# griffin-h/lightcurve_fitting

Measured on AMD Instinct MI355X. Metric: walker-steps/sec (emcee ensemble), higher is better.
Workload: dtype f64

## Files before the change

### lightcurve_fitting_amd/csrc/lcf_device.h

```cpp
#pragma once
#ifndef __HIPCC_RTC__
#include <hip/hip_runtime.h>
#include <stdint.h>
#else
typedef __hip_internal::int32_t int32_t;
typedef __hip_internal::uint32_t uint32_t;
typedef __hip_internal::int64_t int64_t;
typedef __hip_internal::uint64_t uint64_t;
#ifndef INFINITY
#define INFINITY __builtin_huge_valf()
#endif
#endif

namespace lcf {

constexpr int kBlock = 256;
constexpr int kMaxParts = 8;
constexpr int kFewEpochs = 128;
constexpr int kTargetGroups = 4096;
constexpr int kNCoef = 8;
constexpr int kMaxDim = 16;
constexpr int kLdsFiltMax = 64;
constexpr int kLdsTabMax = 3700;
constexpr int kMaxPeers = 8;
// ... 394 lines not shown
                const double Tk = c[1] * exp((2. * eps1 - 0.5) * lt);
                const double E = (c[3] == c[3]) ? exp(fma(alpha, lt, c[3])) : 0.;
                const double L = c[2] * exp(-2. * eps2 * lt - E);
                if (!(L >= 0.)) {
                    pref = qnan();
                } else if (Tk > 0. && Tk < kTmax) {
                    const double i1 = inv_temperature(Tk), i2 = i1 * i1;
                    T = Tk;
                    invT = i1;
                    pref = kC3sq * L * i2 * i2;
                }
            } else if (t < 0. && c[4] != 0.) {
                pref = qnan();
            }
            break;
        }
        case kShockCooling4: {
            const double tt = t / c[3];
            double P1 = 0., P2 = 0., P3 = 0., P4 = 0.;
            if (tt > 0.) {
                const double ltt = log(tt);
                P1 = exp(-4. / 3. * ltt);
                P2 = exp(-0.17 * ltt);
                P3 = exp(-1. / 3. * ltt);
                P4 = exp(-0.45 * ltt);
            }
            const double u = k[1] * t / c[4];
            const double E = u > 0. ? pow(u, k[2]) : 0.;
            const double L = c[2] * (P1 + k[0] * exp(-E) * P2);
            const double Tk = c[1] * fmin(0.97 * P3, P4);
            if (!(L >= 0.)) {
                pref = qnan();
            } else if (Tk > 0. && Tk < kTmax) {
                const double i1 = inv_temperature(Tk), i2 = i1 * i1;
                T = Tk;
                invT = i1;
                pref = kC3sq * L * i2 * i2;
            }
            break;
        }
        case kCompanion:
        case kCompanion2:
        case kCompanion3: {
            if (t > 0.) {
                const double lt = log(t);
                if (lt > -9.5916 && lt < 10.06) {
                    const double Tk = c[1] * exp(-74. / 144. * lt);
                    if (Tk > 0. && Tk < kTmax) {
                        T = Tk;
                        invT = inv_temperature(Tk);
                        pref = c[2] * exp(14. / 9. * lt);
                    }
                }
            }
            break;
        }
        case kBlackbody:
            if (c[1] > 0. && c[1] < kTmax) {
                T = c[1];
                invT = inv_temperature(c[1]);
                pref = c[2];
            } else if (c[2] != c[2]) {
                pref = qnan();
            }
            break;
        default:
            break;
    }
}

#ifndef LCF_TLOG
#define LCF_TLOG 1
#endif
#ifndef LCF_TEXP
#define LCF_TEXP 1
#endif
__device__ inline double tlog(double x) { return LCF_TLOG ? flog(x) : log(x); }

__device__ inline void encode_linear(double invT, double pref, double& x, double& p) {
    x = -invT;
    p = pref;
}

template <class PB>
__device__ __forceinline__ void powerlaw_log_state(const PB& pb, double c3, double c6, double c7, double t,
                                                   const ExpTab et, double& u, double& lp, double& lL) {
    const double* k = pb.consts;
    const double eps1 = k[3], eps2 = k[4], alpha = k[2];
    const double lt = tlog(t);
    const double E = !(c3 == c3) ? 0.
                     : LCF_TEXP ? exp_scaled<true>(fmin(fma(alpha, lt, c3) * kInvLn2N, 1100. * kInvLn2N), et)
                                : exp(fma(alpha, lt, c3));
    lL = fma(-2. * eps2, lt, c7) - E;
    u = fma(2. * eps1 - 0.5, lt, c6);
    lp = fma(-4., u, lL);
}

template <int MODEL = 0>
__device__ inline void thermal_state_log(const DevProblem& pb, const double* __restrict__ c, double t_in, double& x,
                                         double& p, const ExpTab et) {
    const int model = MODEL ? MODEL : pb.model;
    const double t = t_in - c[0];
    x = -0.;
    p = 0.;
    double u = qnan(), lp = 0.;
    switch (model) {
        case kShockCooling:
        case kShockCooling2: {
            if (t > 0.) {
                double lL;
                powerlaw_log_state(pb, c[3], c[6], c[7], t, et, u, lp, lL);
                if (!(lL == lL)) {
                    p = qnan();
                    return;
                }
            } else {
                if (t < 0. && c[4] != 0.) p = qnan();
                return;
            }
            break;
        }
        case kCompanion:
        case kCompanion2:
        case kCompanion3: {
            if (!(t > 0.)) return;
            const double lt = tlog(t);
            if (!(lt > -9.5916 && lt < 10.06)) return;
            u = fma(-74. / 144., lt, c[6]);
            lp = fma(14. / 9., lt, c[7]);
            if (!(lp == lp)) u = qnan();
            break;
        }
        default: {
            double T, invT, pref;
            thermal_state<MODEL>(pb, c, t_in, T, invT, pref);
            if (T > 0. && pref > 0. && pref < INFINITY) {
                u = log(T);
                lp = log(pref);
            } else {
                encode_linear(invT, pref, x, p);
                return;
            }
            break;
        }
    }
    if (!(u == u) || !(u < 34.538776394910684)) return;
    if (lp < -600.) return;
    const double r = (u - pb.itab_u0) * pb.itab_inv_h;
    if (r >= 0. && r < (double)pb.itab_m && lp <= 600.) {
        x = r;
        p = lp;
    } else if (u > -50.) {
        encode_linear(exp(-u), exp(lp), x, p);
    }
}

__device__ __forceinline__ double interp_log_band_sum(const DevProblem& pb, int lds_at, int filt, double r) {
    extern __shared__ __align__(16) unsigned char smem[];
    const int j = (int)r;
    const double s = fma(__builtin_amdgcn_fract(r), 2., -1.);
    double2 q0, q1, q2, q3;
    if (lds_at >= 0) {
        const double2* q = reinterpret_cast<const double2*>(smem + lds_at) + (filt * pb.itab_m * 8 + 8 * j) / 2;
        q0 = q[0], q1 = q[1], q2 = q[2], q3 = q[3];
    } else {
        const double2* q = reinterpret_cast<const double2*>(pb.itab + filt * pb.itab_m * 8 + 8 * j);
        q0 = q[0], q1 = q[1], q2 = q[2], q3 = q[3];
    }
    double g = fma(q0.x, s, q0.y);
    g = fma(g, s, q1.x);
    g = fma(g, s, q1.y);
    g = fma(g, s, q2.x);
// ... 29 lines not shown
```

### lightcurve_fitting_amd/csrc/lcf_hip.hip

```cpp
#include <hip/hip_runtime.h>

#include <algorithm>
#include <chrono>
#include <cmath>
#include <cstdio>
#include <cstdlib>
#include <dlfcn.h>
#include <cstring>
#include <mutex>
#include <numeric>
#include <string>
#include <vector>

#include "lcf.h"
#include "lcf_device.h"
#include "lcf_host.h"
#include "lcf_internal.h"
#include "lcf_keys.h"

#ifndef LCF_KPRE
#define LCF_KPRE 4
#endif
#ifndef LCF_KPRE_SOLO
#define LCF_KPRE_SOLO 2
// ... 311 lines not shown
        double yf[3];
        interp_columns<3, IN_LDS>(pb, itab_at, f, row, s, lnr2k, et, yf);
        const double q0 = (o0.x - yf[0]) * o0.y, q1 = (o1.x - yf[1]) * o1.y, q2 = (o2.x - yf[2]) * o2.y;
        acc = fma(q0, q0, acc);
        acc = fma(q1, q1, acc);
        acc = fma(q2, q2, acc);
    }
    if (f + 2 <= nf) {
        const double2 o0 = yd[(size_t)f * nc], o1 = yd[(size_t)(f + 1) * nc];
        double yf[2];
        interp_columns<2, IN_LDS>(pb, itab_at, f, row, s, lnr2k, et, yf);
        const double q0 = (o0.x - yf[0]) * o0.y, q1 = (o1.x - yf[1]) * o1.y;
        acc = fma(q0, q0, acc);
        acc = fma(q1, q1, acc);
        f += 2;
    }
    if (f < nf) {
        const double2 o0 = yd[(size_t)f * nc];
        double yf[1];
        interp_columns<1, IN_LDS>(pb, itab_at, f, row, s, lnr2k, et, yf);
        const double q0 = (o0.x - yf[0]) * o0.y;
        acc = fma(q0, q0, acc);
    }
    return acc;
}

template <int VARIANT, bool LDS_TAB, int MODEL>
__device__ __forceinline__ double general_column(const DevProblem& pb, const double* __restrict__ p,
                                                  const double* __restrict__ c, const double2* tbase, const FiltDesc* fdesc,
                                                  const ExpTab et, int itab_at, double t_in, int col, bool live, double x,
                                                  double pr) {
    const int nc = pb.em_cols;
    double acc = 0.;
    auto one_point = [&](int k, int filt) {
        const double2 o = pb.em_yd[(size_t)k * nc + col];
        const double yfit = point_model<VARIANT, LDS_TAB, true, MODEL>(pb, c, p, t_in, filt, tbase, fdesc, et, x, pr, itab_at);
        const double r = o.x - yfit;
        if (!MODEL && pb.use_sigma) {
            const double dy = o.y;
            const double su = p[pb.n_dim - 1] * (pb.sigma_abs ? pb.sigma_unit_abs : dy);
            const double var = fma(dy, dy, su * su);
            acc += log(kTwoPi * var) + r * r / var;
        } else {
            const double q = r * o.y;
            acc = fma(q, q, acc);
        }
    };
    if (MODEL || pb.em_dense) {
#pragma unroll 1
        for (int k = 0; k < pb.em_k; ++k)
            if (live) one_point(k, k);
    } else {
#pragma unroll 1
        for (int k = 0; k < pb.em_k; ++k) {
            const int filt = pb.em_filt[(size_t)k * nc + col];
            if (live && filt >= 0) one_point(k, filt);
        }
    }
    return acc;
}

template <int VARIANT, int MODEL>
__device__ __attribute__((noinline)) double cold_column(const DevProblem* pbp, const double* c_mem, const double* p, double t_in,
                                                        int col, bool live, double x, double pr) {
    const DevProblem& pb = *pbp;
    double c[kNCoef];
#pragma unroll
    for (int k = 0; k < kNCoef; ++k) c[k] = c_mem[k];
    return general_column<VARIANT, false, MODEL>(pb, p, c, pb.tab, pb.f_desc, ExpTab{pb.exp2tab}, -1, t_in, col, live, x, pr);
}

template <int VARIANT, int MODEL>
__device__ __attribute__((noinline)) double cold_column_with_state(const DevProblem* pbp, const double* c_mem, const double* p,
                                                                   double t_in, int col, bool live) {
    const DevProblem& pb = *pbp;
    double c[kNCoef], x, pr;
#pragma unroll
    for (int k = 0; k < kNCoef; ++k) c[k] = c_mem[k];
    const ExpTab et{pb.exp2tab};
    thermal_state_log<MODEL>(pb, c, t_in, x, pr, et);
    return general_column<VARIANT, false, MODEL>(pb, p, c, pb.tab, pb.f_desc, et, -1, t_in, col, live, x, pr);
}

template <int MODEL, class PB>
__device__ __forceinline__ bool lean_column(const PB& pb, const double* __restrict__ sc, const ColumnOperands& first,
                                            const ExpTab et, int itab_at, double& acc) {
    const double t = first.t - sc[0];
    double u, lp, lL;
    powerlaw_log_state(pb, sc[3], sc[6], sc[7], t, et, u, lp, lL);
    const double r = (u - pb.itab_u0) * pb.itab_inv_h;
    const bool ok = t > 0. && r >= 0. && r < (double)pb.itab_m && lp >= -600. && lp <= 600.;
    if (__builtin_amdgcn_ballot_w64(!ok) != 0) return false;
    const int row = 8 * (int)r;
    const double s = fma(__builtin_amdgcn_fract(r), 2., -1.);
    acc = fast_column_fetched<true>(pb, itab_at, row, s, lp * kInvLn2N, et, first.o);
    return true;
}
struct ColumnView {
    const double* consts;
    double itab_u0, itab_inv_h;
    int itab_m;
    const double* itab;
};
struct ConstsView {
    const double* consts;
    int model;
};

template <int VARIANT, bool LDS_TAB, bool FETCHED = false, int MODEL = 0, bool COLD = false>
__device__ inline double epochs_loop(const DevProblem& pb, int part, const double* __restrict__ p,
                                     const double* __restrict__ c, const double2* tbase, const FiltDesc* fdesc,
                                     const ExpTab et, int vtid, int itab_at, const ColumnOperands& first = ColumnOperands{},
                                     bool use_first = true, const DevProblem* pb_mem = nullptr,
                                     const double* c_mem = nullptr) {
    part = __builtin_amdgcn_readfirstlane(part);
    const int c0 = part_entry(pb.part_col0, part), c1 = part_entry(pb.part_col0, part + 1);
    const int lane = vtid & 63, v64 = __builtin_amdgcn_readfirstlane(vtid & ~63);
    const bool by_itab = MODEL ? true : VARIANT != 0 && pb.use_itab;
    const bool fast_kind = columns_fast_kind<MODEL>(pb, by_itab);
    const bool companion_fast = !MODEL && LDS_TAB && by_itab && pb.em_dense && pb.itab_uniform && !pb.use_sigma &&
                                pb.model >= kCompanion && pb.model <= kCompanion3 && itab_at >= 0 && pb.n_spl_lds > 0 &&
                                pb.knot_h > 0.;
    const bool ragged_fast = !MODEL && by_itab && !pb.em_dense && pb.itab_uniform && !pb.use_sigma &&
                             (pb.model == kShockCooling || pb.model == kShockCooling2);
    double term = 0.;
    constexpr bool kAhead = MODEL == 0;
    double t_next = 0.;
    if (kAhead && c0 + v64 < c1 && !(FETCHED && use_first)) t_next = pb.em_t[min(c0 + v64 + lane, c1 - 1)];
#pragma unroll 1
    for (int cb = c0 + v64; cb < c1; cb += kBlock) {
        const bool live = cb + lane < c1;
        const int col = live ? cb + lane : c1 - 1;
        const bool fetched = FETCHED && use_first && cb < c0 + kBlock;
        const double t_in = fetched ? first.t : kAhead ? t_next : pb.em_t[col];
        if (kAhead && cb + kBlock < c1) t_next = pb.em_t[min(cb + kBlock + lane, c1 - 1)];
        int filt0 = 0;
        double2 o0 = make_double2(0., 0.);
        if (ragged_fast) {
            filt0 = pb.em_filt[col];
            o0 = pb.em_yd[col];
        }
        double x, pr;
        if (by_itab) {
            thermal_state_log<MODEL>(pb, c, t_in, x, pr, et);
        } else {
            double T;
            thermal_state<MODEL>(pb, c, t_in, T, x, pr);
        }
        LCF_STAMP(0, 13);
        if (ragged_fast && __builtin_amdgcn_ballot_w64(__double2hiint(x) < 0) == 0) {
            const double lnr2k = pr * kInvLn2N;
            const int nc = pb.em_cols;
            double acc = 0.;
#pragma unroll 1
            for (int k = 0; k < pb.em_k; ++k) {
                int filt = filt0;
                double2 o = o0;
                if (k > 0) {
                    filt = pb.em_filt[(size_t)k * nc + col];
                    o = pb.em_yd[(size_t)k * nc + col];
                }
                const double L = interp_log_band_sum(pb, itab_at, max(filt, 0), x);
                const double q = (o.x - exp_scaled<false>(fma(L, kInvLn2N, lnr2k), et)) * o.y;
                acc = filt >= 0 ? fma(q, q, acc) : acc;
            }
            term += live ? acc : 0.;
            continue;
        }
        if (companion_fast && __builtin_amdgcn_ballot_w64(__double2hiint(x) < 0) == 0) {
            const int row = 8 * (int)x;
            const double s = fma(__builtin_amdgcn_fract(x), 2., -1.);
            const double lnr2k = pr * kInvLn2N, inv_s = 1. / c[4];
// ... 447 lines not shown
template <int ND>
__device__ inline void step_body(const DevProblem& pb, const DevSampler& sm, int i, int have_prev, long long prev_row,
                                 int have_next, const DrawRec* __restrict__ draws, const DrawRec* __restrict__ prev_draws,
                                 long long g, int lo, int hi, double* __restrict__ coef, double* __restrict__ lprior) {
    __shared__ double sc[kNCoef + 1];
    const bool mine = i >= lo && i < hi;
    if (threadIdx.x < 64)
        step_serial<ND>(pb, sm, i, true, threadIdx.x, have_prev, prev_row, have_next, draws, prev_draws, g, mine, sc, nullptr,
                        coef, lprior);
}

template <int ND>
__global__ __launch_bounds__(64) void k_step(const DevProblem pb, const DevSampler sm, int have_prev, long long prev_row,
                                             int have_next, const DrawRec* __restrict__ draws,
                                             const DrawRec* __restrict__ prev_draws, long long g, int lo, int hi,
                                             double* __restrict__ coef, double* __restrict__ lprior) {
    step_body<ND>(pb, sm, blockIdx.x, have_prev, prev_row, have_next, draws, prev_draws, g, lo, hi, coef, lprior);
}

constexpr int kFusedScratch = kNCoef + 2 + kMaxDim + (kMaxDim & 1);

__device__ inline double uniform_f64(double v) {
    const long long b = __double_as_longlong(v);
    const int lo = __builtin_amdgcn_readfirstlane((int)(b & 0xffffffffLL));
    const int hi = __builtin_amdgcn_readfirstlane((int)(b >> 32));
    return __longlong_as_double(((long long)hi << 32) | (unsigned int)lo);
}

template <int ND, int VARIANT, bool THERM>
__global__ __launch_bounds__(kBlock, LCF_WAVES) void k_fused(const DevProblem pb, const DevSampler sm, int have_prev,
                                                  long long prev_row, const DrawRec* __restrict__ draws,
                                                  const DrawRec* __restrict__ prev_draws, long long g, int lo, int hi,
                                                  double* __restrict__ lprior) {
    extern __shared__ __align__(16) unsigned char smem[];
    double* exptab = reinterpret_cast<double*>(smem);
    double* red = exptab + kExpTabSize;
    double2* ltab = reinterpret_cast<double2*>(smem + kLdsHead * sizeof(double));
    const FiltDesc* fdesc = reinterpret_cast<const FiltDesc*>(ltab + pb.n_lds_tab);
    const int itab_at = pb.n_itab_lds > 0
                            ? (int)(kLdsHead * sizeof(double) + (pb.n_lds_tab + kFdD2 * pb.n_filters) * sizeof(double2)) : -1;
    double* sc = reinterpret_cast<double*>(ltab + pb.stage_d2);
    double* sq = sc + kNCoef + 2;
    const int tid = threadIdx.x;
    const int n_own = hi - lo;
    if ((int)blockIdx.x >= n_own * pb.n_parts) {
        const int k = ((int)blockIdx.x - n_own * pb.n_parts) * (kBlock / 64) + (tid >> 6);
        const int slot = k < lo ? k : k + n_own;
        if (slot < sm.n_half)
            step_serial<ND>(pb, sm, slot, true, tid & 63, have_prev, prev_row, 1, draws, prev_draws, g, false, nullptr,
                            nullptr, nullptr, nullptr);
        return;
    }
    const int part = blockIdx.x / n_own, i = lo + blockIdx.x % n_own;
    const bool reddened = pb.model == kShockCooling3;
    if (tid < 64)
        step_serial<ND>(pb, sm, i, part == 0, tid, have_prev, prev_row, 1, draws, prev_draws, g, true, sc, sq, nullptr,
                        lprior);
    else if (!reddened)
        stage_tables<VARIANT, true>(pb, exptab, ltab, 0., tid - 64, kBlock - 64);
    __syncthreads();
    if (sc[kNCoef] == -INFINITY) return;
    double cs[kNCoef];
#pragma unroll
    for (int k = 0; k < kNCoef; ++k) cs[k] = uniform_f64(sc[k]);
    if (reddened) stage_tables<VARIANT, true>(pb, exptab, ltab, cs[6], tid, kBlock);
    if (reddened) __syncthreads();
    double term;
    if constexpr (THERM)
        term = epochs_loop<VARIANT, true>(pb, part, sq, cs, ltab, fdesc, ExpTab{exptab}, tid, itab_at);
    else
        term = points_loop<VARIANT, 0, true, false>(pb, part, 0, sq, cs, nullptr, 0, ltab, fdesc, ExpTab{exptab}, nullptr,
                                                    nullptr, tid, itab_at);
    const double psum = store_part_sum(term, red, sm.part2[g & 1] + (size_t)i * part_stride(pb) + part);
    if (sm.n_peers > 0 && tid == 0) mbox_post(sm, g, i, part, part_stride(pb), psum);
}

__device__ inline unsigned long long* board_entry(unsigned long long* board, const DevSampler& sm, unsigned int tag, int wid,
                                                  int col) {
    return board + 2 * ((((size_t)(tag & (unsigned int)(sm.ring - 1)) * sm.n_walkers) + wid) * board_row_entries(sm.n_dim) + col);
}
#ifndef LCF_EARLY_POST
#define LCF_EARLY_POST 0
#endif
__device__ __forceinline__ int not_hoisted(int v) {
    asm volatile("" : "+v"(v));
    return v;
}
__device__ __forceinline__ size_t board_entry_bytes(const RunUniforms& u, unsigned int tag, int wid, int col) {
    return (tag & u.ring_mask) * u.ver_bytes + ((size_t)(unsigned int)wid * u.row_bytes + 16u * (unsigned int)col);
}
__device__ __forceinline__ unsigned long long* board_entry(unsigned long long* board, const RunUniforms& u, unsigned int tag,
                                                           int wid, int col) {
    return reinterpret_cast<unsigned long long*>(reinterpret_cast<unsigned char*>(board) + board_entry_bytes(u, tag, wid, col));
}
__device__ inline unsigned int* board_progress(unsigned long long* board, const DevSampler& sm) {
    return reinterpret_cast<unsigned int*>(reinterpret_cast<unsigned char*>(board) +
                                           board_rows_bytes(sm.ring, sm.n_walkers, sm.n_dim));
}
typedef unsigned int lcf_u32x4 __attribute__((ext_vector_type(4)));
typedef int lcf_i32x4 __attribute__((ext_vector_type(4)));
template <bool AGENT>
__device__ __forceinline__ void store16_past_caches(unsigned long long* p, unsigned long long lo, unsigned long long hi) {
    const lcf_u32x4 v = {(unsigned int)lo, (unsigned int)(lo >> 32), (unsigned int)hi, (unsigned int)(hi >> 32)};
    asm volatile("global_store_dwordx4 %0, %1, off sc0 sc1" : : "v"(p), "v"(v) : "memory");
}
template <bool AGENT>
__device__ __forceinline__ void load16_past_caches(const unsigned long long* p, unsigned long long& lo, unsigned long long& hi) {
    lcf_u32x4 v;
    asm volatile("global_load_dwordx4 %0, %1, off sc0 sc1\n\ts_waitcnt vmcnt(0)" : "=v"(v) : "v"(p) : "memory");
    lo = (unsigned long long)v.x | ((unsigned long long)v.y << 32);
    hi = (unsigned long long)v.z | ((unsigned long long)v.w << 32);
}
template <bool AGENT = false>
__device__ inline void board_post_at(unsigned long long* entry, unsigned int tag, double v) {
    const unsigned long long b = (unsigned long long)__double_as_longlong(v), t = (unsigned long long)tag << 32;
    store16_past_caches<AGENT>(entry, (b & 0xffffffffull) | t, (b >> 32) | t);
}
template <bool AGENT = false>
__device__ inline void board_post(unsigned long long* board, const DevSampler& sm, unsigned int tag, int wid, int col, double v) {
    board_post_at<AGENT>(board_entry(board, sm, tag, wid, col), tag, v);
}
template <bool AGENT = false>
__device__ inline bool board_aborted_at(const unsigned int* flag) {
    return (AGENT ? __hip_atomic_load(flag, __ATOMIC_RELAXED, __HIP_MEMORY_SCOPE_AGENT)
                  : __hip_atomic_load(flag, __ATOMIC_RELAXED, __HIP_MEMORY_SCOPE_SYSTEM)) != 0u;
}
template <bool AGENT = false>
__device__ inline bool board_aborted(const DevSampler& sm) {
    return board_aborted_at<AGENT>(board_progress(sm.board, sm) + kMaxPeers);
}
__device__ inline unsigned int* board_arrivals(const DevSampler& sm) { return board_progress(sm.board, sm) + kMaxPeers + 5; }
__device__ inline void board_abort(const DevSampler& sm, unsigned int what, unsigned int a, unsigned int b, unsigned int c) {
    unsigned int* flag = board_progress(sm.board, sm) + kMaxPeers;
    if (atomicCAS_system(flag, 0u, 1u) == 0u) {
        __hip_atomic_store(flag + 1, what, __ATOMIC_RELAXED, __HIP_MEMORY_SCOPE_SYSTEM);
        __hip_atomic_store(flag + 2, a, __ATOMIC_RELAXED, __HIP_MEMORY_SCOPE_SYSTEM);
        __hip_atomic_store(flag + 3, b, __ATOMIC_RELAXED, __HIP_MEMORY_SCOPE_SYSTEM);
        __hip_atomic_store(flag + 4, c, __ATOMIC_RELAXED, __HIP_MEMORY_SCOPE_SYSTEM);
    }
    atomicOr(sm.err, 2);
    if (sm.snap_flags) sm.snap_flags[kSnapFlags + (blockIdx.x & (kSnapFlags - 1))] = 2u;
}
template <bool AGENT = false>
__device__ inline double board_take_at(const DevSampler& sm, const unsigned long long* p, unsigned int tag, int wid, int col,
                                       unsigned int arrive_goal = 0u) {
    const unsigned long long t0 = wall_clock64();
    bool resident = arrive_goal == 0u;
    for (int spin = 0;; ++spin) {
        unsigned long long a, b;
        load16_past_caches<AGENT>(p, a, b);
        if ((unsigned int)(a >> 32) == tag && (unsigned int)(b >> 32) == tag)
            return __longlong_as_double((long long)((a & 0xffffffffull) | (b << 32)));
        if ((spin & 15) == 15) {
            if (board_aborted<AGENT>(sm)) return qnan();
            if (!resident && wall_clock64() - t0 > sm.resident_ticks) {
                const unsigned int there = __hip_atomic_load(board_arrivals(sm), __ATOMIC_RELAXED, __HIP_MEMORY_SCOPE_AGENT);
                if ((int)(there - arrive_goal) < 0) {
                    board_abort(sm, 3u, tag, (unsigned int)wid, there);
                    return qnan();
                }
                resident = true;
            }
            if (wall_clock64() - t0 > sm.wait_ticks) {
                const bool was_first = !board_aborted<AGENT>(sm);
                board_abort(sm, 1u, tag, (unsigned int)wid, (unsigned int)col);
                if (was_first) {
// ... 162 lines not shown
        x[d] = h.x[d];
        const double cj = h.cj[d];
        q[d] = d < nd ? cj - (cj - x[d]) * dr.z : 0.;
        if (lane == d && d < pb.n_par) arg = q[d];
    }
#ifdef LCF_STAMPS
    asm volatile("s_waitcnt vmcnt(0)" ::: "memory");
#endif
    LCF_STAMP(0, 2);
    const double lg = flog(arg);
#pragma unroll
    for (int d = 0; d < kD; ++d) lq[d] = lane_value(lg, d);
    LCF_STAMP(0, 3);
    double c[kNCoef];
    walker_coefficients<MODEL>(pb, q, lq, c, MODEL ? true : pb.use_itab != 0);
    LCF_STAMP(0, 4);
    double lpr = 0.;
    if (pb.has_priors) {
        double qv = 0.;
#pragma unroll
        for (int d = 0; d < kD; ++d)
            if (lane == d) qv = q[d];
        const double mine = lane < pb.n_dim ? prior_term(my_prior, qv) : 0.;
#pragma unroll
        for (int d = 0; d < kD; ++d)
            if (d < nd) lpr += lane_value(mine, d);
    }
    const double count = BOARD ? lane_value(got, 16 + nd + 1) : 0.;
    if (lane == 0) {
#pragma unroll
        for (int k = 0; k < kNCoef; ++k) sc[k] = c[k];
        sc[kNCoef] = lpr;
#pragma unroll
        for (int d = 0; d < kD; ++d)
            if (d < nd) {
                sq[d] = q[d];
                sx[d] = x[d];
            }
        sx[kMaxDim] = lp_i;
        if (BOARD) sx[kMaxDim + 1] = count;
    }
    LCF_STAMP(0, 5);
}

struct LaneRows {
    double cj, x;
    PriorDev prior;
};

template <int ND, int BOARD>
__device__ __forceinline__ void lane_head_fetch(const DevSampler& sm, const DrawRec& dr, int lane_in, LaneRows& h, long long G,
                                                long long g_run0, unsigned int arrive_goal, const RunUniforms* ru) {
    const int nd = ND > 0 ? ND : __builtin_amdgcn_readfirstlane(ru->nd);
    const int lane = not_hoisted(lane_in);
    h.cj = h.x = 0.;
    if (lane <= nd + 1) {
        const unsigned int wtag = board_tag(G, dr.wage, g_run0), ptag = board_tag(G, dr.page, g_run0);
        const bool both = lane < nd;
        const unsigned int tag_l = both ? ptag : wtag;
        const int wid_l = both ? dr.pid : dr.wid;
        board_take_pair<BOARD == 2>(sm, board_entry(ru->board, *ru, tag_l, wid_l, lane), board_entry(ru->board, *ru, wtag, dr.wid, lane),
                                    tag_l, wtag, wid_l, dr.wid, lane, arrive_goal, h.cj, h.x);
    }
    h.prior = ru->priors[lane & (kMaxDim - 1)];
}

template <int MODEL>
__device__ __attribute__((noinline)) void cold_coefficients(const double* consts, const double* p_mem, double* c_mem, bool write) {
    static_assert(MODEL == kShockCooling, "the model whose coefficients have a branch worth moving out");
    double p[kMaxDim], lq[kMaxDim], c[kNCoef];
#pragma unroll
    for (int d = 0; d < kMaxDim; ++d) p[d] = lq[d] = 0.;
#pragma unroll
    for (int d = 0; d < 5; ++d) p[d] = p_mem[d];
#pragma unroll
    for (int d = 0; d < 4; ++d) lq[d] = flog(p[d]);
    walker_coefficients<MODEL>(ConstsView{consts, MODEL}, p, lq, c, true);
    if (write) {
#pragma unroll
        for (int k = 0; k < kNCoef; ++k) c_mem[k] = c[k];
    }
}

template <int ND, int BOARD, int MODEL>
__device__ __forceinline__ void lane_head(const DevProblem& pb, const DrawRec& dr, int lane_in, double* __restrict__ sc,
                                          double* __restrict__ sq, double* __restrict__ sx, const LaneRows& h,
                                          const RunUniforms* ru) {
    constexpr int kD = ND > 0 ? ND : kMaxDim;
    const int nd = ND > 0 ? ND : __builtin_amdgcn_readfirstlane(ru->nd);
    const int lane = not_hoisted(lane_in);
    const int n_par = ru->n_par, n_dim = ru->n_dim, has_priors = __builtin_amdgcn_readfirstlane(ru->has_priors);
    const double cj = h.cj, x = h.x;
    const double q = lane < nd ? cj - (cj - x) * dr.z : 0.;
#ifdef LCF_STAMPS
    asm volatile("s_waitcnt vmcnt(0)" ::: "memory");
#endif
    LCF_STAMP(0, 2);
    if (lane < nd) sq[lane] = q;
    if (lane <= nd + 1) sx[lane < nd ? lane : lane - nd + kMaxDim] = x;
    const double lg = flog(lane < n_par ? q : 1.);
    double p[kMaxDim], lq[kMaxDim];
#pragma unroll
    for (int d = 0; d < kMaxDim; ++d) p[d] = lq[d] = 0.;
#pragma unroll
    for (int d = 0; d < kD; ++d) {
        p[d] = lane_value(q, d);
        lq[d] = lane_value(lg, d);
    }
    LCF_STAMP(0, 3);
    double c[kNCoef];
    bool c_stored = false;
    if constexpr (MODEL == kShockCooling) {
        const double v = p[0], M = p[1], f = p[2], R = p[3];
        if (v > 0. && M > 0. && f > 0. && R > 0. && v < 1e100 && M < 1e100 && f < 1e100 && R < 1e100) {
            walker_coefficients<MODEL, ConstsView, true>(ConstsView{ru->consts, MODEL}, p, lq, c, true);
        } else {
#pragma unroll
            for (int k = 0; k < kNCoef; ++k) c[k] = 0.;
            cold_coefficients<MODEL>(ru->consts, sq, sc, lane == 0);
            c_stored = true;
        }
    } else {
        walker_coefficients<MODEL>(ConstsView{ru->consts, MODEL ? MODEL : ru->model}, p, lq, c, MODEL ? true : pb.use_itab != 0);
    }
    LCF_STAMP(0, 4);
    double lpr = 0.;
    if (has_priors) {
        const double mine = lane < n_dim ? prior_term(h.prior, q) : 0.;
#pragma unroll
        for (int d = 0; d < kD; ++d)
            if (d < nd) lpr += lane_value(mine, d);
    }
    if (lane == 0) {
        if (!c_stored) {
#pragma unroll
            for (int k = 0; k < kNCoef; k += 2) *reinterpret_cast<double2*>(sc + k) = make_double2(c[k], c[k + 1]);
        }
        sc[kNCoef] = lpr;
    }
    LCF_STAMP(0, 5);
}

constexpr int kSoloScratch = kNCoef + 2 + 2 * (kMaxDim + (kMaxDim & 1));

template <int ND, int VARIANT, bool THERM, int NPARTS, int BOARD, int MODEL>
__device__ __forceinline__ bool solo_half_step(const DevProblem& pb, const DevProblem* __restrict__ pbp, const DevSampler& sm, long long row,
                                               const DrawRec* __restrict__ draws, const DrawRec* draws_next, long long G,
                                               long long g_run0, int i, unsigned char* smem, ColumnOperands& first_col,
                                               bool first, bool write_state, const int tid, const int run_flags = 0,
                                               const unsigned int arrive_goal = 0u, const RunUniforms* ru = nullptr) {
    constexpr bool RES = BOARD >= 2;
    double* exptab = reinterpret_cast<double*>(smem);
    double* red = exptab + kExpTabSize;
    double2* ltab = reinterpret_cast<double2*>(smem + kLdsHead * sizeof(double));
    const FiltDesc* fdesc = RES ? nullptr : reinterpret_cast<const FiltDesc*>(ltab + pb.n_lds_tab);
    int itab_at = -1;
    if constexpr (!RES)
        itab_at = pb.n_itab_lds > 0
                      ? (int)(kLdsHead * sizeof(double) + (pb.n_lds_tab + kFdD2 * pb.n_filters) * sizeof(double2)) : -1;
    double* sc = RES ? reinterpret_cast<double*>(const_cast<RunUniforms*>(ru)) - (kSoloScratch + 4)
                     : reinterpret_cast<double*>(ltab + pb.stage_d2);
    double* sq = sc + kNCoef + 2;
    double* sx = sq + kMaxDim + (kMaxDim & 1);
    int* sctl = reinterpret_cast<int*>(sc + (RES ? kNCoef + 1 : kSoloScratch + 2));
    constexpr int kGroups = NPARTS == 8 ? 4 : 2;
    constexpr int kThreads = kBlock * kGroups;
    constexpr int kD = ND > 0 ? ND : kMaxDim;
    const int nd = ND > 0 ? ND : RES ? __builtin_amdgcn_readfirstlane(ru->nd) : sm.n_dim;
    const bool reddened = !MODEL && (RES ? __builtin_amdgcn_readfirstlane(ru->model) : pb.model) == kShockCooling3;
    LCF_STAMP(0, 0);
#ifdef LCF_STAMPS
    if (tid == 0 && blockIdx.x < 1024) g_wall[((G & 1) * 1024 + blockIdx.x) * 2] = wall_clock64();
#endif
    const DrawRec dr = draws[i];
    if (BOARD == 1 && blockIdx.x == 0 && tid < sm.n_board_ranks)
        __hip_atomic_store(board_progress(sm.peer_board[tid], sm) + sm.board_rank, (unsigned int)G, __ATOMIC_RELAXED,
                           __HIP_MEMORY_SCOPE_SYSTEM);
    if (dr.wid < 0) return false;
    LCF_STAMP(0, 1);
    constexpr bool kFetch = MODEL != 0;
    if (tid < 64) {
        if (BOARD >= 2) __builtin_amdgcn_s_setprio(3);
        if constexpr (RES) {
            LaneRows rows;
            lane_head_fetch<ND, BOARD>(sm, dr, tid, rows, G, g_run0, arrive_goal, ru);
            if (kFetch && first) fetch_column<VARIANT, MODEL>(pb, tid / kBlock, tid % kBlock, first_col);
            lane_head<ND, BOARD, MODEL>(pb, dr, tid, sc, sq, sx, rows, ru);
        } else {
            HeadRows<ND> rows;
            head_fetch<ND, BOARD>(pb, sm, dr, tid, rows, G, g_run0, arrive_goal);
            if (kFetch && first) fetch_column<VARIANT, MODEL>(pb, tid / kBlock, tid % kBlock, first_col);
            proposal_head<ND, BOARD, MODEL>(pb, sm, dr, tid, sc, sq, sx, rows);
        }
        if (BOARD >= 2) __builtin_amdgcn_s_setprio(0);
    } else {
        if (LCF_HEAD_START > 0) __builtin_amdgcn_s_sleep(LCF_HEAD_START);
        if (kFetch && first) fetch_column<VARIANT, MODEL>(pb, tid / kBlock, tid % kBlock, first_col);
        if (BOARD >= 2) {
            if (tid >= 64 && tid < 128 && draws_next != nullptr) {
                const int* nxt = reinterpret_cast<const int*>(draws_next + i);
                int a_, b_;
                asm volatile("s_load_dword %0, %2, 0x0\n\ts_load_dword %1, %2, 0x2c\n\ts_waitcnt lgkmcnt(0)"
                             : "=&s"(a_), "=&s"(b_) : "s"(nxt) : "memory");
            }
        } else if (tid == 64 && draws_next != nullptr) {
            const volatile int* nxt = reinterpret_cast<const volatile int*>(draws_next + i);
            (void)nxt[0];
            (void)nxt[sizeof(DrawRec) / sizeof(int) - 1];
        }
        if (!reddened && first) stage_tables<VARIANT, true>(pb, exptab, ltab, 0., tid - 64, kThreads - 64);
        LCF_STAMP(1, 11);
        if constexpr (RES)
            if (tid == 64) sctl[0] = board_aborted_at<BOARD == 2>(ru->abort_word) ? 1 : 0;
        if (BOARD == 1 && tid < 128) {
            const int lane = tid - 64;
            const unsigned int* progress = board_progress(sm.board, sm);
            const unsigned long long t0 = wall_clock64();
            bool abort = false;
            for (;;) {
                bool ok = true;
                if (G - 2 >= g_run0 && lane < sm.n_board_ranks)
                    ok = (int)(__hip_atomic_load(progress + lane, __ATOMIC_RELAXED, __HIP_MEMORY_SCOPE_SYSTEM) -
                               (unsigned int)(G - 1)) >= 0;
                abort = board_aborted(sm);
                if (__all(ok) || abort) break;
                if (wall_clock64() - t0 > sm.wait_ticks) {
                    board_abort(sm, 2u, (unsigned int)G, (unsigned int)__builtin_ctzll(~__ballot(ok)), 0u);
                    abort = true;
                    break;
                }
                __builtin_amdgcn_s_sleep(2);
            }
            if (lane == 0) sctl[0] = abort ? 1 : 0;
        }
    }
    __syncthreads();
    LCF_STAMP(0, 6);
    double lpr;
    lcf_i32x4 col_group = {0, 0, 0, 0}, col_itab = {0, 0, 0, 0};
    double2 col_grid = make_double2(0., 0.);
    double col_consts[5] = {0., 0., 0., 0., 0.};
    if constexpr (RES) {
        const double2 la = *reinterpret_cast<const double2*>(sc + kNCoef);
        if constexpr (MODEL != 0 && NPARTS <= 2) {
            const int group = __builtin_amdgcn_readfirstlane(not_hoisted(tid) / kBlock);
            col_group = *reinterpret_cast<const lcf_i32x4*>(&ru->group[group]);
            col_grid = *reinterpret_cast<const double2*>(&ru->itab_u0);
            col_itab = *reinterpret_cast<const lcf_i32x4*>(&ru->itab_m);
            const double2 k23 = *reinterpret_cast<const double2*>(&ru->consts[2]);
            col_consts[2] = k23.x, col_consts[3] = k23.y, col_consts[4] = ru->consts[4];
        }
        lpr = la.x;
        if (__builtin_amdgcn_readfirstlane(__double2loint(la.y)) != 0) return true;
    } else {
        if (BOARD && sctl[0] != 0) return true;
        lpr = sc[kNCoef];
    }
    double term = 0.;
    const bool excluded = lpr == -INFINITY;
    bool lean = false;
    if (MODEL != 0 && NPARTS <= 2 && !excluded) {
        const int tid_c = RES ? not_hoisted(tid) : tid;
        const int part = __builtin_amdgcn_readfirstlane(tid_c / kBlock), ltid = tid_c % kBlock;
        int c0, c1;
        if constexpr (RES) {
            c0 = __builtin_amdgcn_readfirstlane(col_group.x);
            c1 = __builtin_amdgcn_readfirstlane(col_group.y);
            lean = first_col.have_o && __builtin_amdgcn_readfirstlane(col_group.z) != 0;
        } else {
            c0 = part_entry(pb.part_col0, part);
            c1 = part_entry(pb.part_col0, part + 1);
            lean = first_col.have_o && itab_at >= 0 && c1 - c0 <= kBlock && part < pb.n_parts;
        }
        if (lean) {
            LCF_STAMP(0, 7);
            double acc = 0.;
            if (c0 + (ltid & ~63) < c1) {
                const bool live = c0 + ltid < c1;
                bool in_grid;
                if constexpr (RES)
                    in_grid = lean_column<MODEL>(ColumnView{col_consts, col_grid.x, col_grid.y, col_itab.x, nullptr}, sc, first_col,
                                                 ExpTab{exptab}, col_itab.y, acc);
                else
                    in_grid = lean_column<MODEL>(pb, sc, first_col, ExpTab{exptab}, itab_at, acc);
                if (!in_grid)
                    acc = cold_column_with_state<VARIANT, MODEL>(pbp, sc, sq, first_col.t, min(c0 + ltid, c1 - 1), live);
                term = live ? acc : 0.;
            }
            LCF_STAMP(0, 8);
            LCF_STAMP(1, 12);
            const double ws = wave_sum(term);
            if ((tid & 63) == 0) red[tid_c >> 6] = ws;
        }
    }
    if (!excluded && !lean) {
        double cs[kNCoef];
#pragma unroll
        for (int k = 0; k < kNCoef; ++k) cs[k] = uniform_f64(sc[k]);
        if constexpr (RES) {
            fdesc = reinterpret_cast<const FiltDesc*>(ltab + pb.n_lds_tab);
            itab_at = __builtin_amdgcn_readfirstlane(ru->itab_at);
        }
        if (reddened) stage_tables<VARIANT, true>(pb, exptab, ltab, cs[6], tid, kThreads);
        const int part = tid / kBlock, ltid = tid % kBlock;
        if (reddened) __syncthreads();
        LCF_STAMP(0, 7);
        if (NPARTS > 2) {
#pragma unroll 1
            for (int pp = part; pp < pb.n_parts; pp += kGroups) {
                term = epochs_loop<VARIANT, true, kFetch, MODEL, true>(pb, pp, sq, cs, ltab, fdesc, ExpTab{exptab}, ltid, itab_at,
                                                                       first_col, pp == part, pbp, sc);
                const double ws = wave_sum(term);
                if ((tid & 63) == 0) red[4 * pp + (ltid >> 6)] = ws;
            }
        } else {
            if (part < pb.n_parts)
                term = epochs_loop<VARIANT, true, kFetch, MODEL, true>(pb, part, sq, cs, ltab, fdesc, ExpTab{exptab}, ltid, itab_at,
                                                                       first_col, true, pbp, sc);
            LCF_STAMP(0, 8);
            LCF_STAMP(1, 12);
            const double ws = wave_sum(term);
            if ((tid & 63) == 0) red[tid >> 6] = ws;
        }
    }
    size_t entry_early = 0;
    if constexpr (RES && LCF_EARLY_POST != 0)
        if (tid < 64) entry_early = board_entry_bytes(*ru, (unsigned int)(G + 1), dr.wid, not_hoisted(tid));
    __syncthreads();
    LCF_STAMP(0, 9);
    if (BOARD) {
        if (tid >= 64) return false;
        if (BOARD >= 2) __builtin_amdgcn_s_setprio(3);
        if constexpr (RES) {
            const double2* red2 = reinterpret_cast<const double2*>(red);
            const double2 lc = *reinterpret_cast<const double2*>(sx + kMaxDim);
            const int col = not_hoisted(tid);
            const int mine = col < nd ? col : 0;
            const double q_mine = sq[mine], x_mine = sx[mine];
            const double sum0 = ru->sum0;
            const unsigned int tag = (unsigned int)(G + 1);
            const size_t entry = LCF_EARLY_POST != 0 ? entry_early : board_entry_bytes(*ru, tag, dr.wid, col);
            unsigned char* const own_board = reinterpret_cast<unsigned char*>(ru->board);
            double sum = sum0;
            if (NPARTS <= 2) {
                const int n_parts = ru->n_parts;
                const double2 a0 = red2[0], a1 = red2[1], b0 = red2[2], b1 = red2[3];
                const double s1 = sum + ((a0.x + a0.y) + (a1.x + a1.y));
                sum = n_parts > 0 ? s1 : sum;
                const double s2 = sum + ((b0.x + b0.y) + (b1.x + b1.y));
                sum = n_parts > 1 ? s2 : sum;
            } else {
                const int n_parts = __builtin_amdgcn_readfirstlane(ru->n_parts);
                for (int k = 0; k < n_parts; ++k) sum += (red2[2 * k].x + red2[2 * k].y) + (red2[2 * k + 1].x + red2[2 * k + 1].y);
            }
            const double scored = lpr - 0.5 * sum;
            const double nlp = excluded ? -INFINITY : scored;
            const double lp_i = lc.x;
            const bool ok = (dr.zl + nlp - lp_i) > dr.lnu;
            const double count = lc.y + (ok ? 1. : 0.);
            if (tid <= nd + 1) {
                const double v = tid < nd ? (ok ? q_mine : x_mine) : tid == nd ? (ok ? nlp : lp_i) : count;
                if (BOARD == 2) {
                    board_post_at<true>(reinterpret_cast<unsigned long long*>(own_board + entry), tag, v);
// ... 2358 lines not shown
```

Baseline: 101.2 million.

## Compute lean-column log(t - t0) early in non-head waves after extra barrier

In model-specialised resident kernels with few parts, the head wave publishes the walker's proposal coordinates to shared memory, and an extra barrier then lets the other waves read t_0. Those waves compute log(t - t0) for the lean column while the head wave finishes its coefficient work, taking the log off the critical path. The power-law state routine gains a flag to accept a precomputed log. Wave 0, the head wave, still computes its own log late. The cost is an additional __syncthreads per step, a reordered abort-flag store, and a dependence on t_0 being a fixed coordinate index per model.

```diff
diff --git a/lightcurve_fitting_amd/csrc/lcf_device.h b/lightcurve_fitting_amd/csrc/lcf_device.h
--- a/lightcurve_fitting_amd/csrc/lcf_device.h
+++ b/lightcurve_fitting_amd/csrc/lcf_device.h
@@ -500,12 +500,12 @@
     p = pref;
 }
 
-template <class PB>
+template <bool HAVE_LT = false, class PB>
 __device__ __forceinline__ void powerlaw_log_state(const PB& pb, double c3, double c6, double c7, double t,
                                                    const ExpTab et, double& u, double& lp, double& lL) {
     const double* k = pb.consts;
     const double eps1 = k[3], eps2 = k[4], alpha = k[2];
-    const double lt = tlog(t);
+    const double lt = HAVE_LT ? t : tlog(t);
     const double E = !(c3 == c3) ? 0.
                      : LCF_TEXP ? exp_scaled<true>(fmin(fma(alpha, lt, c3) * kInvLn2N, 1100. * kInvLn2N), et)
                                 : exp(fma(alpha, lt, c3));
diff --git a/lightcurve_fitting_amd/csrc/lcf_hip.hip b/lightcurve_fitting_amd/csrc/lcf_hip.hip
--- a/lightcurve_fitting_amd/csrc/lcf_hip.hip
+++ b/lightcurve_fitting_amd/csrc/lcf_hip.hip
@@ -417,12 +417,12 @@
     return general_column<VARIANT, false, MODEL>(pb, p, c, pb.tab, pb.f_desc, et, -1, t_in, col, live, x, pr);
 }
 
-template <int MODEL, class PB>
+template <int MODEL, bool HAVE_LT = false, class PB>
 __device__ __forceinline__ bool lean_column(const PB& pb, const double* __restrict__ sc, const ColumnOperands& first,
-                                            const ExpTab et, int itab_at, double& acc) {
+                                            const ExpTab et, int itab_at, double& acc, double lt = 0.) {
     const double t = first.t - sc[0];
     double u, lp, lL;
-    powerlaw_log_state(pb, sc[3], sc[6], sc[7], t, et, u, lp, lL);
+    powerlaw_log_state<HAVE_LT>(pb, sc[3], sc[6], sc[7], HAVE_LT ? lt : t, et, u, lp, lL);
     const double r = (u - pb.itab_u0) * pb.itab_inv_h;
     const bool ok = t > 0. && r >= 0. && r < (double)pb.itab_m && lp >= -600. && lp <= 600.;
     if (__builtin_amdgcn_ballot_w64(!ok) != 0) return false;
@@ -1036,6 +1036,9 @@
 #ifndef LCF_EARLY_POST
 #define LCF_EARLY_POST 0
 #endif
+#ifndef LCF_EARLY_LOG
+#define LCF_EARLY_LOG 1
+#endif
 __device__ __forceinline__ int not_hoisted(int v) {
     asm volatile("" : "+v"(v));
     return v;
@@ -1364,7 +1367,7 @@
     }
 }
 
-template <int ND, int BOARD, int MODEL>
+template <int ND, int BOARD, int MODEL, bool EARLY = false>
 __device__ __forceinline__ void lane_head(const DevProblem& pb, const DrawRec& dr, int lane_in, double* __restrict__ sc,
                                           double* __restrict__ sq, double* __restrict__ sx, const LaneRows& h,
                                           const RunUniforms* ru) {
@@ -1379,6 +1382,7 @@
 #endif
     LCF_STAMP(0, 2);
     if (lane < nd) sq[lane] = q;
+    if constexpr (EARLY) __syncthreads();
     if (lane <= nd + 1) sx[lane < nd ? lane : lane - nd + kMaxDim] = x;
     const double lg = flog(lane < n_par ? q : 1.);
     double p[kMaxDim], lq[kMaxDim];
@@ -1461,13 +1465,17 @@
     if (dr.wid < 0) return false;
     LCF_STAMP(0, 1);
     constexpr bool kFetch = MODEL != 0;
+    constexpr bool kEarly = RES && MODEL != 0 && NPARTS <= 2 && LCF_EARLY_LOG != 0;
+    constexpr int kT0 = MODEL == kShockCooling ? 4 : MODEL == kShockCooling2 ? 3 : -1;
+    static_assert(!kEarly || kT0 >= 0, "a model-specialised resident kernel names the coordinate that is t_0");
+    double lt_early = 0.;
     if (tid < 64) {
         if (BOARD >= 2) __builtin_amdgcn_s_setprio(3);
         if constexpr (RES) {
             LaneRows rows;
             lane_head_fetch<ND, BOARD>(sm, dr, tid, rows, G, g_run0, arrive_goal, ru);
             if (kFetch && first) fetch_column<VARIANT, MODEL>(pb, tid / kBlock, tid % kBlock, first_col);
-            lane_head<ND, BOARD, MODEL>(pb, dr, tid, sc, sq, sx, rows, ru);
+            lane_head<ND, BOARD, MODEL, kEarly>(pb, dr, tid, sc, sq, sx, rows, ru);
         } else {
             HeadRows<ND> rows;
             head_fetch<ND, BOARD>(pb, sm, dr, tid, rows, G, g_run0, arrive_goal);
@@ -1490,10 +1498,18 @@
             (void)nxt[0];
             (void)nxt[sizeof(DrawRec) / sizeof(int) - 1];
         }
+        if constexpr (RES)
+            if (tid == 64) sctl[0] = board_aborted_at<BOARD == 2>(ru->abort_word) ? 1 : 0;
+        if constexpr (kEarly) {
+            const int tid_e = not_hoisted(tid);
+            const bool lean_e = __builtin_amdgcn_readfirstlane(ru->group[__builtin_amdgcn_readfirstlane(tid_e / kBlock)].lean) != 0;
+            const bool mine = lean_e && first_col.have_o;
+            __syncthreads();
+            const double t0 = sq[kT0];
+            if (mine) lt_early = tlog(first_col.t - t0);
+        }
         if (!reddened && first) stage_tables<VARIANT, true>(pb, exptab, ltab, 0., tid - 64, kThreads - 64);
         LCF_STAMP(1, 11);
-        if constexpr (RES)
-            if (tid == 64) sctl[0] = board_aborted_at<BOARD == 2>(ru->abort_word) ? 1 : 0;
         if (BOARD == 1 && tid < 128) {
             const int lane = tid - 64;
             const unsigned int* progress = board_progress(sm.board, sm);
@@ -1560,7 +1576,12 @@
             if (c0 + (ltid & ~63) < c1) {
                 const bool live = c0 + ltid < c1;
                 bool in_grid;
-                if constexpr (RES)
+                if constexpr (kEarly) {
+                    if (__builtin_amdgcn_readfirstlane(tid_c >> 6) == 0)
+                        lt_early = tlog(first_col.t - sc[0]);
+                    in_grid = lean_column<MODEL, true>(ColumnView{col_consts, col_grid.x, col_grid.y, col_itab.x, nullptr}, sc,
+                                                       first_col, ExpTab{exptab}, col_itab.y, acc, lt_early);
+                } else if constexpr (RES)
                     in_grid = lean_column<MODEL>(ColumnView{col_consts, col_grid.x, col_grid.y, col_itab.x, nullptr}, sc, first_col,
                                                  ExpTab{exptab}, col_itab.y, acc);
                 else
```

Measured after the change: 105.0 million (median of 6 runs). 3.8% higher.
